# lipku/LiveTalking

Hardware: NVIDIA H100
Metric: lip-sync frames/sec (wav2lip256, 256x256, batch 16, mel + U-Net fwd + paste-back) (higher is better)
Workload: dtype f16 (fp32 accumulate); mel f64; paste u8

## Files before the change

### livetalking_b200/csrc/conv_halo.cu

```cuda
#include <cuda.h>

#include <atomic>
#include <mutex>
#include <utility>

#include "conv_halo.h"
#include "ltb_internal.h"
#include "ptx_sm90.cuh"

#ifdef LTB_HALO_DIAG
#include <cstdlib>
#define LTB_DIAG(bit) (p.dbg & (bit))
#else
#define LTB_DIAG(bit) 0
#endif

namespace ltb {

constexpr int kHaloP = 10;
constexpr int kHaloThreads = 384;
constexpr int kProducerRegs = 40, kConsumerRegs = 232;
constexpr int kSms = 132;

template <int BN, int NSUB, int NACC, int TAPS, int RC = 0>
// ... 477 lines not shown
          bool row_ok = false;
          const size_t opix = halo_pix(img, ty, tx, q >> 1, 0, wq * 16 + (lane >> 2) + 8 * (q & 1), row_ok);
          if (q < 2 * NSUB && row_ok) {
            float ha0 = head_sw[96], ha1 = head_sw[97], ha2 = head_sw[98];
#pragma unroll
            for (int i = 0; i < 4; ++i)
#pragma unroll
              for (int src = 0; src < 4; ++src) {
                const float2 f = __half22float2(*reinterpret_cast<__half2*>(&hv[src][i]));
                const int cc = 8 * i + 2 * src;
                ha0 = fmaf(f.x, head_sw[cc], ha0);
                ha0 = fmaf(f.y, head_sw[cc + 1], ha0);
                ha1 = fmaf(f.x, head_sw[32 + cc], ha1);
                ha1 = fmaf(f.y, head_sw[32 + cc + 1], ha1);
                ha2 = fmaf(f.x, head_sw[64 + cc], ha2);
                ha2 = fmaf(f.y, head_sw[64 + cc + 1], ha2);
              }
            float* o = p.head_out + opix * 3;
            o[0] = (1.f / (1.f + expf(-ha0))) * 255.f;
            o[1] = (1.f / (1.f + expf(-ha1))) * 255.f;
            o[2] = (1.f / (1.f + expf(-ha2))) * 255.f;
          }
        }
      }
    }
  }

  __syncthreads();
  if (gn_smem) {
    for (int i = tid; i < p.gn_images * p.gn_groups * 2; i += kHaloThreads) {
      const float v = gn_acc[i];
      if (v != 0.f) atomicAdd(p.gn_stats + i, v);
    }
  }
}

typedef CUresult (*EncodeTiledFn)(CUtensorMap*, CUtensorMapDataType, cuuint32_t, void*, const cuuint64_t*, const cuuint64_t*,
                                  const cuuint32_t*, const cuuint32_t*, CUtensorMapInterleave, CUtensorMapSwizzle,
                                  CUtensorMapL2promotion, CUtensorMapFloatOOBfill);

static EncodeTiledFn get_encode() {
  static EncodeTiledFn fn = nullptr;
  static std::once_flag once;
  std::call_once(once, []() {
    void* p = nullptr;
    cudaDriverEntryPointQueryResult q;
    if (cudaGetDriverEntryPoint("cuTensorMapEncodeTiled", &p, cudaEnableDefault, &q) == cudaSuccess &&
        q == cudaDriverEntryPointSuccess)
      fn = reinterpret_cast<EncodeTiledFn>(p);
  });
  return fn;
}

static bool encode(CUtensorMap* tm, int rank, const void* base, const cuuint64_t* dims, const cuuint64_t* strides_bytes,
                   const cuuint32_t* box, int spatial_stride = 1) {
  EncodeTiledFn fn = get_encode();
  if (!fn) return false;
  cuuint32_t es[5] = {1, (cuuint32_t)spatial_stride, (cuuint32_t)spatial_stride, 1, 1};
  return fn(tm, CU_TENSOR_MAP_DATA_TYPE_FLOAT16, (cuuint32_t)rank, const_cast<void*>(base), dims, strides_bytes, box, es,
            CU_TENSOR_MAP_INTERLEAVE_NONE, CU_TENSOR_MAP_SWIZZLE_128B, CU_TENSOR_MAP_L2_PROMOTION_L2_256B,
            CU_TENSOR_MAP_FLOAT_OOB_FILL_NONE) == CUDA_SUCCESS;
}

static bool is_conv3x3(const ConvParams& p) {
  if (p.nphases != 1 || p.ph[0].ntaps != 9 || p.sy != 1 || p.sx != 1 || p.osy != 1 || p.osx != 1) return false;
  for (int t = 0; t < 9; ++t)
    if (p.ph[0].dy[t] != t / 3 - 1 || p.ph[0].dx[t] != t % 3 - 1) return false;
  return p.IH == p.GH && p.IW == p.GW && p.OH == p.GH && p.OW == p.GW;
}
static bool is_convT(const ConvParams& p) {
  if (p.nphases != 4 || p.osy != 2 || p.osx != 2 || p.sy != 1 || p.sx != 1) return false;
  const int nt[4] = {1, 2, 2, 4};
  for (int i = 0; i < 4; ++i)
    if (p.ph[i].ntaps != nt[i]) return false;
  return p.IH == p.GH && p.IW == p.GW && p.OH == 2 * p.GH && p.OW == 2 * p.GW;
}

static bool is_conv3x3_s2(const ConvParams& p) {
  if (p.nphases != 1 || p.ph[0].ntaps != 9 || p.sy != 2 || p.sx != 2 || p.osy != 1 || p.osx != 1) return false;
  for (int t = 0; t < 9; ++t)
    if (p.ph[0].dy[t] != t / 3 - 1 || p.ph[0].dx[t] != t % 3 - 1) return false;
  return p.IH == 2 * p.GH && p.IW == 2 * p.GW && p.OH == p.GH && p.OW == p.GW;
}

static bool is_upconv(const ConvParams& p) {
  return p.upconv == 1 && p.nphases == 4 && p.osy == 2 && p.osx == 2 && p.sy == 1 && p.sx == 1 && p.IH == p.GH && p.IW == p.GW &&
         p.OH == 2 * p.GH && p.OW == 2 * p.GW;
}

static bool is_gemm(const ConvParams& p) {
  return p.nphases == 1 && p.ph[0].ntaps == 1 && p.ph[0].dy[0] == 0 && p.ph[0].dx[0] == 0 && p.sy == 1 && p.sx == 1 && p.osy == 1 &&
         p.osx == 1 && p.IH == p.GH && p.IW == p.GW && p.OH == p.GH && p.OW == p.GW;
}

static bool pick_cfg(const ConvParams& p, int* BN, int* NSUB, int* NACC);

bool conv_halo_supported(const ConvParams& p) {
  if (p.zbatch > 1) return false;
  if ((p.OCtot % 8) || (p.oc_off % 8) || (reinterpret_cast<uintptr_t>(p.out) % 16)) return false;
  if (p.res && ((p.RCtot % 8) || (p.rc_off % 8) || (reinterpret_cast<uintptr_t>(p.res) % 16))) return false;
  if (p.group_slot && (!is_gemm(p) || (p.w_slot_stride * 2) % 16 != 0)) return false;
  if (is_gemm(p)) {
    return p.Cout % 32 == 0 && p.Cin % 8 == 0 && p.Cin >= 32 && (p.ICtot % 8) == 0 && (p.ic_off % 8) == 0 && (p.Ktot % 8) == 0 &&
           (p.ph[0].koff % 8) == 0 && p.M >= 512 && get_encode() != nullptr;
  }
  if (is_conv3x3_s2(p)) {
    return p.Cout % 32 == 0 && p.Cin >= 64 && (p.ICtot % 8) == 0 && (p.ic_off % 8) == 0 && p.Ktot == 9 * p.Cin && p.GH >= 16 &&
           p.GW >= 8 && get_encode() != nullptr;
// ... 32 lines not shown
  if (is_conv3x3_s2(p)) {
    *NACC = 1;
    *NSUB = 1;
    *BN = (p.Cout % 64 == 0) ? 64 : 32;
    return true;
  }
  const bool tr = is_convT(p);
  *NACC = tr ? 4 : 1;
  if (tr) {
    *NSUB = 1;
    *BN = (p.Cout % 64 == 0) ? 64 : 32;
    return true;
  }
  const long ksteps = (p.Cin + 15) / 16;
  double best = 1e30;
  for (int bn : {128, 64, 32}) {
    if (p.Cout % bn) continue;
    for (int nsub : {2, 1}) {
      if (nsub == 2 && (p.GH % 32) != 0) continue;
      const long tiles = (long)p.N * ((p.GH + 16 * nsub - 1) / (16 * nsub)) * ((p.GW + 7) / 8) * (p.Cout / bn);
      const long waves = (tiles + kSms - 1) / kSms;
      const double tile = (double)ksteps * 9 * nsub * (55.0 + 0.2 * bn) + 800.0;
      const double epi = (waves == 1) ? 40.0 * nsub * bn : 0.0;
      const double cost = waves * tile + epi;
      if (cost < best * 0.9) {
        best = cost;
        *BN = bn;
        *NSUB = nsub;
      }
    }
  }
  return best < 1e30;
}

int conv_halo_make_plan(const ConvParams& p, const __half* w_tap_major, HaloPlan* out) {
  if (!conv_halo_supported(p)) return 1;
  HaloParams& h = out->hp;
  std::memset(&h, 0, sizeof(h));
  out->grouped = false;
  int BN, NSUB, NACC;
  if (!pick_cfg(p, &BN, &NSUB, &NACC)) return 1;
  out->BN = BN;
  out->NSUB = NSUB;
  out->NACC = NACC;
  const bool up = is_upconv(p);
  const bool s2 = is_conv3x3_s2(p);
  const bool tr = NACC == 4 && !up;
  const bool gemm = is_gemm(p);
  out->TAPS = gemm ? 1 : (up ? 16 : (s2 ? 10 : 9));
  if (gemm) {
    cuuint64_t dims[2] = {(cuuint64_t)p.Cin, (cuuint64_t)p.M};
    cuuint64_t strides[1] = {(cuuint64_t)p.ICtot * 2};
    cuuint32_t box[2] = {64, (cuuint32_t)(128 * NSUB)};
    if (!encode(&h.tm_in, 2, p.in + p.ic_off, dims, strides, box)) return 2;
    cuuint64_t wdims[3] = {(cuuint64_t)p.Cin, (cuuint64_t)p.Cout, (cuuint64_t)p.slots};
    cuuint64_t wstrides[2] = {(cuuint64_t)p.Ktot * 2, (cuuint64_t)p.w_slot_stride * 2};
    cuuint32_t wbox[3] = {64, (cuuint32_t)BN, 1};
    if (!encode(&h.tm_w, p.group_slot ? 3 : 2, p.w + p.ph[0].koff, wdims, wstrides, wbox)) return 2;
  } else
  {
    cuuint64_t dims[4] = {(cuuint64_t)p.Cin, (cuuint64_t)p.IW, (cuuint64_t)p.IH, (cuuint64_t)p.N};
    cuuint64_t strides[3] = {(cuuint64_t)p.ICtot * 2, (cuuint64_t)p.IW * p.ICtot * 2, (cuuint64_t)p.IH * p.IW * p.ICtot * 2};
    cuuint32_t box[4] = {64, (cuuint32_t)kHaloP, (cuuint32_t)(16 * NSUB + 2), 1};
    if (s2) {
      box[1] = 2 * 9 - 1;
      box[2] = 2 * (16 * NSUB + 1) - 1;
    }
    if (!encode(&h.tm_in, 4, p.in + p.ic_off, dims, strides, box, s2 ? 2 : 1)) return 2;
  }
  if (up) {
    cuuint64_t dims[3] = {(cuuint64_t)p.Cin, (cuuint64_t)p.Cout, 16};
    cuuint64_t strides[2] = {(cuuint64_t)p.Cin * 2, (cuuint64_t)p.Cout * p.Cin * 2};
    cuuint32_t box[3] = {64, (cuuint32_t)BN, 4};
    if (!encode(&h.tm_w, 3, w_tap_major, dims, strides, box)) return 2;
  } else if (!gemm) {
    cuuint64_t dims[3] = {(cuuint64_t)p.Cin, (cuuint64_t)p.Cout, 9};
    cuuint64_t strides[2] = {(cuuint64_t)p.Cin * 2, (cuuint64_t)p.Cout * p.Cin * 2};
    cuuint32_t box[3] = {64, (cuuint32_t)BN, 3};
    if (!encode(&h.tm_w, 3, w_tap_major, dims, strides, box)) return 2;
  }
  h.out = p.out;
  h.res = p.res;
  h.bias = p.bias;
  h.N = p.N;
  h.M = p.M;
  h.Cin = p.Cin;
  h.gn_stats = nullptr;
#ifdef LTB_HALO_DIAG
  if (const char* e = std::getenv("LTB_HALO_DIAG")) h.dbg = std::atoi(e);
#endif
  h.OCtot = p.OCtot;
  h.oc_off = p.oc_off;
  h.RCtot = p.RCtot;
  h.rc_off = p.rc_off;
  h.OH = p.OH;
  h.OW = p.OW;
  h.GH = p.GH;
  h.GW = p.GW;
  h.osy = p.osy;
  h.osx = p.osx;
  h.relu = p.relu;
  h.res_halo = halo_res_smem_ok(BN, NSUB, NACC, out->TAPS) && p.res != nullptr && p.res == p.in && p.Cin == p.Cout &&
               p.rc_off == p.ic_off && p.RCtot == p.ICtot;
  h.halo_y0 = tr ? 0 : -1;
  h.halo_x0 = tr ? 0 : -1;
  if (up || tr) {
    const int slot_phase[4] = {0, 1, 3, 2};
    for (int sl = 0; sl < 4; ++sl) {
      h.acc_oy[sl] = p.ph[slot_phase[sl]].ooy;
      h.acc_ox[sl] = p.ph[slot_phase[sl]].oox;
    }
  } else {
    h.acc_oy[0] = p.ph[0].ooy;
    h.acc_ox[0] = p.ph[0].oox;
  }
  h.tiles_n = p.Cout / BN;
  if (gemm) {
    h.halo_y0 = h.halo_x0 = 0;
    h.tiles_x = (p.M + 128 * NSUB - 1) / (128 * NSUB);
    if (p.group_slot) {
      out->grouped = true;
      h.group_slot = p.group_slot;
      h.group_rows = p.group_images * p.GH * p.GW;
      h.group_tiles = (h.group_rows + 128 * NSUB - 1) / (128 * NSUB);
      h.bias_slot_stride = p.bias_slot_stride;
      h.tiles_x = (p.N / p.group_images) * h.group_tiles;
    }
    h.tiles_y = 1;
    h.total_tiles = h.tiles_x * h.tiles_n;
    return 0;
  }
  h.tiles_x = (p.GW + 7) / 8;
// ... 129 lines not shown
```

### livetalking_b200/csrc/conv_halo.h

```cpp
#pragma once
#include <cuda.h>
#include <cuda_runtime.h>

#include <cstring>

#include "conv_params.h"

namespace ltb {

struct alignas(64) HaloParams {
  CUtensorMap tm_in;
  CUtensorMap tm_w;
  __half* out;
  const __half* res;
  const float* bias;
  int N, M, Cin;
  int OCtot, oc_off, RCtot, rc_off;
  int OH, OW, osy, osx;
  int GH, GW;
  int relu;
  int res_halo;
  int halo_y0, halo_x0;
  int acc_oy[4], acc_ox[4];
  int tiles_x, tiles_y, tiles_n, total_tiles;
  float* gn_stats;
  int gn_groups, gn_cpg, gn_hw, gn_images;
  const float* head_w;
  const float* head_b;
  float* head_out;
  const int* group_slot;
  int group_rows, group_tiles;
  long long bias_slot_stride;
#ifdef LTB_HALO_DIAG
  int dbg;
#endif
};

struct HaloPlan {
  HaloParams hp;
  int BN, NSUB, NACC, TAPS;
  bool grouped;
};

bool conv_halo_supported(const ConvParams& p);
int conv_halo_make_plan(const ConvParams& p, const __half* w_tap_major, HaloPlan* out);
cudaError_t launch_conv_halo(const HaloPlan& pl, cudaStream_t st);
int conv_halo_sms();
int conv_halo_resident_chunks(const HaloPlan& pl, int sms);
bool conv_halo_gn_fusable(const HaloPlan& pl, int cout_total, int groups, int hw);
cudaError_t launch_w_tap_major(const __half* w, __half* wt, int cout, int cin, cudaStream_t st, int ntaps = 9);
cudaError_t launch_w_tap_major_convT(const __half* w, __half* wt, int cout, int cin, cudaStream_t st);

}
```

### livetalking_b200/csrc/conv_plan.cu

```cuda
#include <cstring>
#include <string>
#include <vector>

#include "../../include/ltb200.h"
#include "conv_plan.h"
#include "ltb_internal.h"

namespace ltb {

static const int kTd[2][2] = {{0, 0}, {0, 1}};
static const int kTk[2][2] = {{1, 0}, {2, 0}};
static const int kTn[2] = {1, 2};
static const int kUd[2][2] = {{-1, 0}, {0, 1}};

ConvParams conv_params(ConvMode mode, int N, ConvSlice in, int IH, int IW, int Cin, ConvSlice out, int OH, int OW, int Cout,
                       ConvSlice res, const __half* w, int Ktot, int w_koff, const float* bias, bool relu, ConvTaps taps) {
  ConvParams p;
  std::memset(&p, 0, sizeof(p));
  p.in = in.p;
  p.N = N;
  p.IH = IH;
  p.IW = IW;
  p.ICtot = in.Ctot;
  p.ic_off = in.off;
// ... 8 lines not shown
  p.Cout = Cout;
  p.res = res.p;
  p.RCtot = res.Ctot;
  p.rc_off = res.off;
  p.w = w;
  p.Ktot = Ktot;
  p.bias = bias;
  p.relu = relu ? 1 : 0;
  if (mode == ConvMode::Dense) {
    p.sy = taps.sy;
    p.sx = taps.sx;
    p.GH = OH;
    p.GW = OW;
    p.nphases = 1;
    ConvPhase& ph = p.ph[0];
    ph.ntaps = taps.KH * taps.KW;
    ph.koff = w_koff;
    for (int kh = 0; kh < taps.KH; ++kh)
      for (int kw = 0; kw < taps.KW; ++kw) {
        ph.dy[kh * taps.KW + kw] = (signed char)(kh - taps.pad_t);
        ph.dx[kh * taps.KW + kw] = (signed char)(kw - taps.pad_l);
      }
  } else {
    const bool up = mode == ConvMode::Upsample2x;
    p.GH = IH;
    p.GW = IW;
    p.osy = p.osx = 2;
    p.nphases = 4;
    p.upconv = up ? 1 : 0;
    int koff = w_koff;
    for (int a = 0; a < 2; ++a)
      for (int b = 0; b < 2; ++b) {
        ConvPhase& ph = p.ph[a * 2 + b];
        const int na = up ? 2 : kTn[a], nb = up ? 2 : kTn[b];
        ph.ntaps = na * nb;
        ph.koff = koff;
        ph.ooy = a;
        ph.oox = b;
        for (int i = 0; i < na; ++i)
          for (int j = 0; j < nb; ++j) {
            ph.dy[i * nb + j] = (signed char)(up ? kUd[a][i] : kTd[a][i]);
            ph.dx[i * nb + j] = (signed char)(up ? kUd[b][j] : kTd[b][j]);
          }
        koff += ph.ntaps * Cin;
      }
  }
  p.M = N * p.GH * p.GW;
  return p;
}

int conv_plan(const ConvParams& p, const __half* w_tap, ConvPath path, ConvPlan* out) {
  out->p = p;
  out->halo = false;
  if (p.group_slot) {
    if (p.group_images < 1 || p.N % p.group_images || p.slots < 1 || p.w_slot_stride < 0 || p.bias_slot_stride < 0)
      return LTB_FAIL("conv: grouped weights need N divisible by group_images >= 1, slots >= 1 and non-negative slot strides");
    if (p.zbatch > 1 || p.upconv) return LTB_FAIL("conv: grouped weights cannot be combined with zbatch or the fused upsample");
  }
  if (path == ConvPath::Gather) return 0;
  const bool gemm = p.nphases == 1 && p.ph[0].ntaps == 1;
  if (!((w_tap || gemm) && conv_halo_supported(p))) {
    if (path == ConvPath::Auto) return 0;
    return LTB_FAIL("conv: the halo kernel cannot run " + std::to_string(p.N) + "x" + std::to_string(p.IH) + "x" + std::to_string(p.IW) +
                    "x" + std::to_string(p.Cin) + " -> " + std::to_string(p.OH) + "x" + std::to_string(p.OW) + "x" + std::to_string(p.Cout) +
                    (w_tap || gemm ? "" : " without tap-major weights"));
  }
  if (conv_halo_make_plan(p, w_tap, &out->hp) != 0) return LTB_FAIL("conv: halo plan / tensor map creation failed");
  out->halo = true;
  return 0;
}

cudaError_t conv_launch(const ConvPlan& pl, cudaStream_t st, float* splitk_ws, size_t ws_floats) {
  return pl.halo ? launch_conv_halo(pl.hp, st) : launch_conv_gather(pl.p, st, splitk_ws, ws_floats);
}

bool conv_plan_variant(const ConvPlan& pl, bool have_ws, size_t ws_floats, ltb_conv_variant* out) {
  std::memset(out, 0, sizeof(*out));
  out->grouped = pl.p.group_slot != nullptr;
  if (pl.halo) {
    out->kernel = 1;
    out->taps = pl.hp.TAPS;
    out->bn = pl.hp.BN;
    out->nsub = pl.hp.NSUB;
    out->nacc = pl.hp.NACC;
    out->resident_chunks = conv_halo_resident_chunks(pl.hp, conv_halo_sms());
    out->res_halo = pl.hp.hp.res_halo;
    return true;
  }
  int ksplit = 0;
  if (!conv_gather_pick(pl.p, have_ws, ws_floats, &out->bn, &out->kb, &ksplit)) return false;
  out->ksplit = ksplit > 1 ? ksplit : 1;
  return true;
}

bool conv_plan_fuse_gn_stats(ConvPlan* pl, float* stats, int groups, int hw) {
  const ConvParams& p = pl->p;
  if (!pl->halo || pl->hp.grouped || p.oc_off != 0 || p.OCtot != p.Cout || !conv_halo_gn_fusable(pl->hp, p.Cout, groups, hw)) return false;
  HaloParams& h = pl->hp.hp;
  h.gn_stats = stats;
  h.gn_groups = groups;
  h.gn_cpg = p.Cout / groups;
  h.gn_hw = hw;
  h.gn_images = p.M / hw;
  return true;
}

bool conv_plan_fuse_head(ConvPlan* pl, const float* w, const float* b, float* out) {
  if (!pl->halo || pl->hp.grouped || pl->hp.BN != 32 || pl->p.Cout != 32) return false;
  pl->hp.hp.head_w = w;
  pl->hp.hp.head_b = b;
  pl->hp.hp.head_out = out;
  return true;
}

static void pack_conv_w(const float* w, int cout, int cin, int KH, int KW, std::vector<__half>& out) {
  out.resize((size_t)cout * KH * KW * cin);
  for (int co = 0; co < cout; ++co)
    for (int kh = 0; kh < KH; ++kh)
      for (int kw = 0; kw < KW; ++kw)
        for (int ci = 0; ci < cin; ++ci)
          out[((size_t)co * KH * KW + kh * KW + kw) * cin + ci] = __float2half(w[(((size_t)co * cin + ci) * KH + kh) * KW + kw]);
}
static void pack_convT_w(const float* w, int cin, int cout, std::vector<__half>& out) {
  out.resize((size_t)cout * 9 * cin);
  for (int co = 0; co < cout; ++co) {
    size_t k = 0;
    for (int a = 0; a < 2; ++a)
      for (int b = 0; b < 2; ++b)
        for (int i = 0; i < kTn[a]; ++i)
          for (int j = 0; j < kTn[b]; ++j) {
            const int kh = kTk[a][i], kw = kTk[b][j];
// ... 28 lines not shown
  }
  if (OH <= 0 || OW <= 0) return LTB_FAIL("empty output");
  const size_t in_b = (size_t)d->N * d->IH * d->IW * d->Cin * 2, out_b = (size_t)d->N * OH * OW * d->Cout * 2;
  __half *din = nullptr, *dout = nullptr, *dw = nullptr, *dres = nullptr, *dwt = nullptr;
  float* dbias = nullptr;
  float* dws = nullptr;
  cudaEvent_t e0 = nullptr, e1 = nullptr;
  int rc = 0;
  auto cleanup = [&]() {
    cudaFree(din);
    cudaFree(dout);
    cudaFree(dw);
    cudaFree(dres);
    cudaFree(dwt);
    cudaFree(dws);
    cudaFree(dbias);
    if (e0) cudaEventDestroy(e0);
    if (e1) cudaEventDestroy(e1);
  };
#define CK(x)                                                             \
  do {                                                                    \
    cudaError_t _e = (x);                                                 \
    if (_e != cudaSuccess) {                                              \
      rc = LTB_FAIL(std::string(#x) + ": " + cudaGetErrorString(_e));     \
      cleanup();                                                          \
      return rc;                                                          \
    }                                                                     \
  } while (0)
  CK(cudaMalloc(&din, in_b));
  CK(cudaMalloc(&dout, out_b));
  CK(cudaMalloc(&dw, wp.size() * 2));
  CK(cudaMalloc(&dbias, (size_t)d->Cout * 4));
  CK(cudaMemcpy(din, in_f16, in_b, cudaMemcpyHostToDevice));
  CK(cudaMemcpy(dw, wp.data(), wp.size() * 2, cudaMemcpyHostToDevice));
  CK(cudaMemcpy(dbias, bias_f32, (size_t)d->Cout * 4, cudaMemcpyHostToDevice));
  CK(cudaMemset(dout, 0xFF, out_b));
  if (d->has_res) {
    CK(cudaMalloc(&dres, out_b));
    CK(cudaMemcpy(dres, res_f16, out_b, cudaMemcpyHostToDevice));
  }
  if (d->KH == 3 && d->KW == 3) {
    CK(cudaMalloc(&dwt, wp.size() * 2));
    CK(d->transposed ? launch_w_tap_major_convT(dw, dwt, d->Cout, d->Cin, nullptr) : launch_w_tap_major(dw, dwt, d->Cout, d->Cin, nullptr));
  }
  const ConvParams p = conv_params(d->transposed ? ConvMode::Transposed : ConvMode::Dense, d->N, {din, d->Cin, 0}, d->IH, d->IW, d->Cin,
                                   {dout, d->Cout, 0}, OH, OW, d->Cout, d->has_res ? ConvSlice{dres, d->Cout, 0} : ConvSlice{}, dw, Ktot, 0,
                                   dbias, d->relu != 0, {d->KH, d->KW, d->sy, d->sx, d->pad, d->pad});
  const ConvPath path = d->force_path == 1 ? ConvPath::Gather : d->force_path == 2 ? ConvPath::Halo : ConvPath::Auto;
  ConvPlan pl;
  if (conv_plan(p, dwt, path, &pl)) {
    cleanup();
    return 1;
  }
  const size_t ws_floats = pl.halo ? 0 : (size_t)1 << 22;
  if (ws_floats) {
    CK(cudaMalloc(&dws, ws_floats * sizeof(float)));
    CK(cudaMemset(dws, 0, ws_floats * sizeof(float)));
  }
  CK(conv_launch(pl, nullptr, dws, ws_floats));
  if (reps > 0) {
    CK(cudaEventCreate(&e0));
    CK(cudaEventCreate(&e1));
    for (int i = 0; i < 3; ++i) CK(conv_launch(pl, nullptr, dws, ws_floats));
    CK(cudaEventRecord(e0, nullptr));
    for (int i = 0; i < reps; ++i) CK(conv_launch(pl, nullptr, dws, ws_floats));
    CK(cudaEventRecord(e1, nullptr));
    CK(cudaEventSynchronize(e1));
    CK(cudaEventElapsedTime(ms_out, e0, e1));
    *ms_out /= reps;
  }
  CK(cudaDeviceSynchronize());
  CK(cudaMemcpy(out_f16, dout, out_b, cudaMemcpyDeviceToHost));
#undef CK
  cleanup();
  return 0;
}

extern "C" {

int ltb_conv2d_f16(const ltb_conv_desc* d, const void* in_f16, const float* w_f32, const float* bias_f32,
                   const void* res_f16, void* out_f16) {
  return conv2d_f16_impl(d, in_f16, w_f32, bias_f32, res_f16, out_f16, 0, nullptr);
}

int ltb_conv2d_f16_timed(const ltb_conv_desc* d, const void* in_f16, const float* w_f32, const float* bias_f32,
                         const void* res_f16, void* out_f16, int reps, float* ms_per_launch) {
  if (reps < 1 || !ms_per_launch) return LTB_FAIL("conv2d_f16_timed: reps >= 1 and a result pointer are required");
  return conv2d_f16_impl(d, in_f16, w_f32, bias_f32, res_f16, out_f16, reps, ms_per_launch);
}

}
```

### livetalking_b200/csrc/conv_plan.h

```cpp
#pragma once
#include <cuda_runtime.h>

#include "conv_halo.h"

struct ltb_conv_variant;

namespace ltb {

struct ConvSlice {
  const __half* p;
  int Ctot, off;
};

enum class ConvMode {
  Dense,
  Transposed,
  Upsample2x,
};
struct ConvTaps {
  int KH, KW, sy, sx, pad_t, pad_l;
};

inline int conv_out_dim(int in, int k, int s, int pad) { return (in + 2 * pad - k) / s + 1; }

ConvParams conv_params(ConvMode mode, int N, ConvSlice in, int IH, int IW, int Cin, ConvSlice out, int OH, int OW, int Cout,
                       ConvSlice res, const __half* w, int Ktot, int w_koff, const float* bias, bool relu, ConvTaps taps = {});

enum class ConvPath {
  Auto,
  Gather,
  Halo,
};
struct ConvPlan {
  ConvParams p{};
  bool halo = false;
  HaloPlan hp{};
};

int conv_plan(const ConvParams& p, const __half* w_tap, ConvPath path, ConvPlan* out);
cudaError_t conv_launch(const ConvPlan& pl, cudaStream_t st, float* splitk_ws, size_t ws_floats);
bool conv_plan_variant(const ConvPlan& pl, bool have_ws, size_t ws_floats, ltb_conv_variant* out);

bool conv_plan_fuse_gn_stats(ConvPlan* pl, float* stats, int groups, int hw);
bool conv_plan_fuse_head(ConvPlan* pl, const float* w, const float* b, float* out);

}
```

### livetalking_b200/csrc/ptx_sm90.cuh

```cuda
#pragma once
#include <cuda_fp16.h>
#include <cstdint>
#include <cstdio>

namespace ltb {

__device__ __forceinline__ uint32_t smem_u32(const void* p) {
  return static_cast<uint32_t>(__cvta_generic_to_shared(p));
}

__device__ __forceinline__ void mbar_init(uint32_t bar, uint32_t count) {
  asm volatile("mbarrier.init.shared::cta.b64 [%0], %1;" ::"r"(bar), "r"(count) : "memory");
}
__device__ __forceinline__ void mbar_fence_init() {
  asm volatile("fence.mbarrier_init.release.cluster;" ::: "memory");
}
__device__ __forceinline__ void mbar_arrive(uint32_t bar) {
  asm volatile("mbarrier.arrive.shared::cta.b64 _, [%0];" ::"r"(bar) : "memory");
}
__device__ __forceinline__ void mbar_arrive_expect_tx(uint32_t bar, uint32_t bytes) {
  asm volatile("mbarrier.arrive.expect_tx.shared::cta.b64 _, [%0], %1;" ::"r"(bar), "r"(bytes) : "memory");
}
__device__ __forceinline__ bool mbar_try_wait(uint32_t bar, uint32_t parity) {
  uint32_t ok;
// ... 18 lines not shown
  asm volatile("fence.proxy.async.shared::cta;" ::: "memory");
}

__device__ __forceinline__ void cp_async16(uint32_t dst, const void* src, uint32_t src_bytes) {
  asm volatile("cp.async.cg.shared.global [%0], [%1], 16, %2;" ::"r"(dst), "l"(src), "r"(src_bytes) : "memory");
}
__device__ __forceinline__ void cp_async_commit() { asm volatile("cp.async.commit_group;" ::: "memory"); }
template <int N>
__device__ __forceinline__ void cp_async_wait() {
  asm volatile("cp.async.wait_group %0;" ::"n"(N) : "memory");
}
__device__ __forceinline__ uint4 lds128(uint32_t addr) {
  uint4 v;
  asm volatile("ld.shared.v4.u32 {%0, %1, %2, %3}, [%4];" : "=r"(v.x), "=r"(v.y), "=r"(v.z), "=r"(v.w) : "r"(addr) : "memory");
  return v;
}

__device__ __forceinline__ void tma_prefetch_desc(const void* tmap) {
  asm volatile("prefetch.tensormap [%0];" ::"l"(tmap) : "memory");
}
__device__ __forceinline__ void tma_load_2d(uint32_t dst, const void* tmap, uint32_t bar, int c0, int c1) {
  asm volatile(
      "cp.async.bulk.tensor.2d.shared::cluster.global.mbarrier::complete_tx::bytes [%0], [%1, {%3, %4}], [%2];" ::"r"(dst),
      "l"(tmap), "r"(bar), "r"(c0), "r"(c1)
      : "memory");
}
__device__ __forceinline__ void tma_load_3d(uint32_t dst, const void* tmap, uint32_t bar, int c0, int c1, int c2) {
  asm volatile(
      "cp.async.bulk.tensor.3d.shared::cluster.global.mbarrier::complete_tx::bytes [%0], [%1, {%3, %4, %5}], [%2];" ::"r"(dst),
      "l"(tmap), "r"(bar), "r"(c0), "r"(c1), "r"(c2)
      : "memory");
}
__device__ __forceinline__ void tma_load_4d(uint32_t dst, const void* tmap, uint32_t bar, int c0, int c1, int c2, int c3) {
  asm volatile(
      "cp.async.bulk.tensor.4d.shared::cluster.global.mbarrier::complete_tx::bytes [%0], [%1, {%3, %4, %5, %6}], [%2];" ::"r"(
          dst),
      "l"(tmap), "r"(bar), "r"(c0), "r"(c1), "r"(c2), "r"(c3)
      : "memory");
}
__device__ __forceinline__ void tma_load_5d(uint32_t dst, const void* tmap, uint32_t bar, int c0, int c1, int c2, int c3,
                                            int c4) {
  asm volatile(
      "cp.async.bulk.tensor.5d.shared::cluster.global.mbarrier::complete_tx::bytes [%0], [%1, {%3, %4, %5, %6, %7}], [%2];" ::
          "r"(dst),
      "l"(tmap), "r"(bar), "r"(c0), "r"(c1), "r"(c2), "r"(c3), "r"(c4)
      : "memory");
}

__device__ __forceinline__ void ldmatrix_x4(uint32_t& r0, uint32_t& r1, uint32_t& r2, uint32_t& r3, uint32_t saddr) {
  asm volatile("ldmatrix.sync.aligned.m8n8.x4.shared.b16 {%0, %1, %2, %3}, [%4];"
               : "=r"(r0), "=r"(r1), "=r"(r2), "=r"(r3)
               : "r"(saddr)
               : "memory");
}

__device__ __forceinline__ uint64_t wgmma_desc(uint32_t saddr, uint32_t lbo_bytes, uint32_t sbo_bytes, uint32_t layout) {
  uint64_t d = 0;
  d |= (uint64_t)((saddr & 0x3FFFF) >> 4);
  d |= (uint64_t)((lbo_bytes >> 4) & 0x3FFF) << 16;
  d |= (uint64_t)((sbo_bytes >> 4) & 0x3FFF) << 32;
  d |= (uint64_t)(layout & 3) << 62;
  return d;
}
__host__ __device__ constexpr uint32_t wgmma_hi_128b(uint32_t sbo_bytes) { return (sbo_bytes >> 4) | (1u << 30); }
__device__ __forceinline__ uint32_t wgmma_lo(uint32_t saddr) { return ((saddr & 0x3FFFFu) >> 4) | (1u << 16); }
__device__ __forceinline__ uint64_t wgmma_lohi(uint32_t lo, uint32_t hi) { return ((uint64_t)hi << 32) | lo; }

__device__ __forceinline__ void wgmma_fence() { asm volatile("wgmma.fence.sync.aligned;" ::: "memory"); }
__device__ __forceinline__ void wgmma_commit() { asm volatile("wgmma.commit_group.sync.aligned;" ::: "memory"); }
template <int N>
__device__ __forceinline__ void wgmma_wait() {
  asm volatile("wgmma.wait_group.sync.aligned %0;" ::"n"(N) : "memory");
}
template <int R>
__device__ __forceinline__ void wgmma_fence_regs(float (&d)[R]) {
#pragma unroll
  for (int i = 0; i < R; ++i) asm volatile("" : "+f"(d[i])::"memory");
}

template <int N>
struct Wgmma;
#define LTB_D1(i) "+f"(d[i])
#define LTB_D2(i) LTB_D1(i), LTB_D1(i + 1)
#define LTB_D4(i) LTB_D2(i), LTB_D2(i + 2)
#define LTB_D8(i) LTB_D4(i), LTB_D4(i + 4)
#define LTB_D16(i) LTB_D8(i), LTB_D8(i + 8)
#define LTB_D32(i) LTB_D16(i), LTB_D16(i + 16)
#define LTB_D64(i) LTB_D32(i), LTB_D32(i + 32)
#define LTB_D128(i) LTB_D64(i), LTB_D64(i + 64)
#define LTB_WG_HEAD(P) "{\n.reg .pred p;\nsetp.ne.b32 p, %" P ", 0;\nwgmma.mma_async.sync.aligned.m64n"
#define LTB_WG_SS(N, REGS, A, B, P) LTB_WG_HEAD(P) N "k16.f32.f16.f16 " REGS ", %" A ", %" B ", p, 1, 1, 0, 0;\n}\n"
#define LTB_WG_RS(N, REGS, A, B, P) \
  LTB_WG_HEAD(P) N "k16.f32.f16.f16 " REGS ", {%" A "}, %" B ", p, 1, 1, 0;\n}\n"

template <>
struct Wgmma<16> {
#define LTB_R "{%0,%1,%2,%3,%4,%5,%6,%7}"
  __device__ __forceinline__ static void ss(float (&d)[8], uint64_t a, uint64_t b, uint32_t acc) {
    asm volatile(LTB_WG_SS("16", LTB_R, "8", "9", "10") : LTB_D8(0) : "l"(a), "l"(b), "r"(acc));
  }
  __device__ __forceinline__ static void rs(float (&d)[8], const uint32_t (&a)[4], uint64_t b, uint32_t acc) {
    asm volatile(LTB_WG_RS("16", LTB_R, "8,%9,%10,%11", "12", "13") : LTB_D8(0)
                 : "r"(a[0]), "r"(a[1]), "r"(a[2]), "r"(a[3]), "l"(b), "r"(acc));
  }
#undef LTB_R
};
// ... 162 lines not shown
```

### livetalking_b200/csrc/w2l_engine.cu

```cuda
#include <cstring>
#include <memory>
#include <mutex>
#include <string>
#include <vector>

#include "../../include/ltb200.h"
#include "conv_plan.h"
#include "ltb_internal.h"
#include "stem_umma.h"

namespace ltb {

static thread_local std::string g_last_error;
void set_error(const std::string& msg) { g_last_error = msg; }

bool pdl_default() {
  static const bool on = [] {
    const char* e = std::getenv("LTB_NO_PDL");
    return !(e && e[0] && e[0] != '0');
  }();
  return on;
}
static thread_local int g_pdl = -1;
bool pdl_enabled() { return g_pdl < 0 ? pdl_default() : g_pdl == 1; }
// ... 240 lines not shown
  const int catS[8] = {512, 512, 512, 256, 128, 64, 32, 16};
  __half* cat[8];
  for (int i = 0; i < 8; ++i) {
    void* p;
    if (dev_alloc(s, (size_t)B * catH[i] * catH[i] * (catD[i] + catS[i]) * 2, &p, true)) return 1;
    cat[i] = static_cast<__half*>(p);
  }
  const size_t tmp_bytes = (size_t)B * 256 * 256 * 64 * 2;
  __half* ring[2] = {nullptr, nullptr};
  int ring_next = 0;
  auto new_tmp = [&](int H, int W, int C, View* v) -> int {
    void* p = nullptr;
    if (keep) {
      if (dev_alloc(s, (size_t)B * H * W * C * 2, &p, true)) return 1;
    } else {
      if (!ring[ring_next]) {
        if (dev_alloc(s, tmp_bytes, &p, true)) return 1;
        ring[ring_next] = static_cast<__half*>(p);
      }
      p = ring[ring_next];
      ring_next ^= 1;
    }
    *v = View{static_cast<__half*>(p), H, W, C, 0, C};
    return 0;
  };
  __half* aring[2] = {nullptr, nullptr};
  int aring_next = 0;
  auto new_atmp = [&](int H, int W, int C, View* v) -> int {
    void* p = nullptr;
    if (keep) {
      if (dev_alloc(s, (size_t)B * H * W * C * 2, &p, true)) return 1;
    } else {
      if (!aring[aring_next]) {
        if (dev_alloc(s, (size_t)B * 80 * 16 * 32 * 2, &p, true)) return 1;
        aring[aring_next] = static_cast<__half*>(p);
      }
      p = aring[aring_next];
      aring_next ^= 1;
    }
    *v = View{static_cast<__half*>(p), H, W, C, 0, C};
    return 0;
  };
  auto cat_dec = [&](int i) { return View{cat[i], catH[i], catH[i], catD[i] + catS[i], 0, catD[i]}; };
  auto cat_skip = [&](int i) { return View{cat[i], catH[i], catH[i], catD[i] + catS[i], catD[i], catS[i]}; };
  auto cat_all = [&](int i) { return View{cat[i], catH[i], catH[i], catD[i] + catS[i], 0, catD[i] + catS[i]}; };

  auto record = [&](int li, const View& v) {
    s->louts[li] = LayerOut{v.p, v.H, v.W, v.C, v.Ctot, v.c_off};
  };
  const ConvPath path = (s->flags & LTB_SESSION_NO_HALO) ? ConvPath::Gather : ConvPath::Auto;
  auto push_conv = [&](int li, const ConvParams& p) -> int {
    Op o;
    if (conv_plan(p, m->wt[li], path, &o.conv)) return LTB_FAIL("plan: layer " + std::to_string(li) + ": " + g_last_error);
    o.type = o.conv.halo ? 4 : 0;
    s->ops.push_back(o);
    return 0;
  };
  auto add_conv = [&](int li, const View& in, const View& out, const View* res) -> int {
    const LDef& L = kLayers[li];
    if (in.C != L.cin || out.C != L.cout) return LTB_FAIL("plan: channel mismatch at layer " + std::to_string(li));
    const int OH = conv_out_dim(in.H, L.k, L.sy, L.pad), OW = conv_out_dim(in.W, L.k, L.sx, L.pad);
    if (OH != out.H || OW != out.W) return LTB_FAIL("plan: spatial mismatch at layer " + std::to_string(li));
    const ConvParams p = conv_params(ConvMode::Dense, B, in.slice(), in.H, in.W, L.cin, out.slice(), OH, OW, L.cout,
                                     res ? res->slice() : ConvSlice{}, m->w[li], L.k * L.k * L.cin, 0, m->bias[li], true,
                                     {L.k, L.k, L.sy, L.sx, L.pad, L.pad});
    if (push_conv(li, p)) return 1;
    record(li, out);
    return 0;
  };
  auto add_convT = [&](int li, const View& in, const View& out) -> int {
    const LDef& L = kLayers[li];
    if (in.C != L.cin || out.C != L.cout || out.H != 2 * in.H) return LTB_FAIL("plan: convT mismatch at layer " + std::to_string(li));
    const ConvParams p = conv_params(ConvMode::Transposed, B, in.slice(), in.H, in.W, L.cin, out.slice(), out.H, out.W, L.cout,
                                     ConvSlice{}, m->w[li], 9 * L.cin, 0, m->bias[li], true);
    if (push_conv(li, p)) return 1;
    record(li, out);
    return 0;
  };

  {
    Op o;
    o.type = 6;
    o.branch = 1;
    s->ops.push_back(o);
  }
  View a_prev;
  if (new_atmp(80, 16, 32, &a_prev)) return 1;
  {
    Op o;
    o.type = 2;
    o.audio_out = a_prev.p;
    o.branch = 1;
    s->ops.push_back(o);
    record(0, a_prev);
  }
  {
    int H = 80, W = 16;
    for (int li = 1; li <= 12; ++li) {
      const LDef& L = kLayers[li];
      const int OH = conv_out_dim(H, L.k, L.sy, L.pad), OW = conv_out_dim(W, L.k, L.sx, L.pad);
      View o;
      if (new_atmp(OH, OW, L.cout, &o)) return 1;
      if (add_conv(li, a_prev, o, L.res ? &a_prev : nullptr)) return 1;
      s->ops.back().branch = 1;
      a_prev = o;
      H = OH;
      W = OW;
// ... 750 lines not shown
```

Before: 6880.

## Add ping-pong warpgroup kernel for 64-channel residual 3x3 convs

Adds a specialized persistent kernel for stride-1 3x3 convolutions with 64 input and output channels and an in-place residual. Two consumer warpgroups alternate tiles, ordered by named barriers, so one warpgroup's epilogue overlaps the other's WGMMA. The weights stay resident in shared memory, inputs come through a 4-stage TMA ring, and outputs are written back with TMA stores after stmatrix. The residual is read from the halo tile already in shared memory rather than from global memory. It is on by default for eligible layers and adds a new code path with tight shape constraints and custom synchronisation that must be correct.

```diff
diff --git a/livetalking_b200/csrc/conv_halo.cu b/livetalking_b200/csrc/conv_halo.cu
--- a/livetalking_b200/csrc/conv_halo.cu
+++ b/livetalking_b200/csrc/conv_halo.cu
@@ -553,8 +553,8 @@
   return fn;
 }
 
-static bool encode(CUtensorMap* tm, int rank, const void* base, const cuuint64_t* dims, const cuuint64_t* strides_bytes,
-                   const cuuint32_t* box, int spatial_stride = 1) {
+bool encode_tmap_f16(CUtensorMap* tm, int rank, const void* base, const cuuint64_t* dims, const cuuint64_t* strides_bytes,
+                     const cuuint32_t* box, int spatial_stride) {
   EncodeTiledFn fn = get_encode();
   if (!fn) return false;
   cuuint32_t es[5] = {1, (cuuint32_t)spatial_stride, (cuuint32_t)spatial_stride, 1, 1};
@@ -693,11 +693,11 @@
     cuuint64_t dims[2] = {(cuuint64_t)p.Cin, (cuuint64_t)p.M};
     cuuint64_t strides[1] = {(cuuint64_t)p.ICtot * 2};
     cuuint32_t box[2] = {64, (cuuint32_t)(128 * NSUB)};
-    if (!encode(&h.tm_in, 2, p.in + p.ic_off, dims, strides, box)) return 2;
+    if (!encode_tmap_f16(&h.tm_in, 2, p.in + p.ic_off, dims, strides, box)) return 2;
     cuuint64_t wdims[3] = {(cuuint64_t)p.Cin, (cuuint64_t)p.Cout, (cuuint64_t)p.slots};
     cuuint64_t wstrides[2] = {(cuuint64_t)p.Ktot * 2, (cuuint64_t)p.w_slot_stride * 2};
     cuuint32_t wbox[3] = {64, (cuuint32_t)BN, 1};
-    if (!encode(&h.tm_w, p.group_slot ? 3 : 2, p.w + p.ph[0].koff, wdims, wstrides, wbox)) return 2;
+    if (!encode_tmap_f16(&h.tm_w, p.group_slot ? 3 : 2, p.w + p.ph[0].koff, wdims, wstrides, wbox)) return 2;
   } else
   {
     cuuint64_t dims[4] = {(cuuint64_t)p.Cin, (cuuint64_t)p.IW, (cuuint64_t)p.IH, (cuuint64_t)p.N};
@@ -707,18 +707,18 @@
       box[1] = 2 * 9 - 1;
       box[2] = 2 * (16 * NSUB + 1) - 1;
     }
-    if (!encode(&h.tm_in, 4, p.in + p.ic_off, dims, strides, box, s2 ? 2 : 1)) return 2;
+    if (!encode_tmap_f16(&h.tm_in, 4, p.in + p.ic_off, dims, strides, box, s2 ? 2 : 1)) return 2;
   }
   if (up) {
     cuuint64_t dims[3] = {(cuuint64_t)p.Cin, (cuuint64_t)p.Cout, 16};
     cuuint64_t strides[2] = {(cuuint64_t)p.Cin * 2, (cuuint64_t)p.Cout * p.Cin * 2};
     cuuint32_t box[3] = {64, (cuuint32_t)BN, 4};
-    if (!encode(&h.tm_w, 3, w_tap_major, dims, strides, box)) return 2;
+    if (!encode_tmap_f16(&h.tm_w, 3, w_tap_major, dims, strides, box)) return 2;
   } else if (!gemm) {
     cuuint64_t dims[3] = {(cuuint64_t)p.Cin, (cuuint64_t)p.Cout, 9};
     cuuint64_t strides[2] = {(cuuint64_t)p.Cin * 2, (cuuint64_t)p.Cout * p.Cin * 2};
     cuuint32_t box[3] = {64, (cuuint32_t)BN, 3};
-    if (!encode(&h.tm_w, 3, w_tap_major, dims, strides, box)) return 2;
+    if (!encode_tmap_f16(&h.tm_w, 3, w_tap_major, dims, strides, box)) return 2;
   }
   h.out = p.out;
   h.res = p.res;
diff --git a/livetalking_b200/csrc/conv_halo.h b/livetalking_b200/csrc/conv_halo.h
--- a/livetalking_b200/csrc/conv_halo.h
+++ b/livetalking_b200/csrc/conv_halo.h
@@ -45,6 +45,8 @@
 bool conv_halo_supported(const ConvParams& p);
 int conv_halo_make_plan(const ConvParams& p, const __half* w_tap_major, HaloPlan* out);
 cudaError_t launch_conv_halo(const HaloPlan& pl, cudaStream_t st);
+bool encode_tmap_f16(CUtensorMap* tm, int rank, const void* base, const cuuint64_t* dims, const cuuint64_t* strides_bytes,
+                     const cuuint32_t* box, int spatial_stride = 1);
 int conv_halo_sms();
 int conv_halo_resident_chunks(const HaloPlan& pl, int sms);
 bool conv_halo_gn_fusable(const HaloPlan& pl, int cout_total, int groups, int hw);
diff --git a/livetalking_b200/csrc/conv_pingpong.cu b/livetalking_b200/csrc/conv_pingpong.cu
--- /dev/null
+++ b/livetalking_b200/csrc/conv_pingpong.cu
@@ -0,0 +1,210 @@
+#include <cuda.h>
+
+#include <cstdlib>
+#include <cstring>
+
+#include "conv_halo.h"
+#include "conv_pingpong.h"
+#include "ltb_internal.h"
+#include "ptx_sm90.cuh"
+
+namespace ltb {
+
+namespace {
+
+constexpr int kThreads = 384;
+constexpr int kProducerRegs = 40, kConsumerRegs = 232;
+constexpr int kP = 10, kHR = 18;
+constexpr int kStages = 4;
+constexpr int kABytesRaw = kHR * kP * 128;
+constexpr int kABytes = (kABytesRaw + 1023) & ~1023;
+constexpr int kTapBytes = 64 * 128;
+constexpr int kWBytes = 9 * kTapBytes;
+constexpr int kOutBytes = 128 * 128;
+constexpr int kSmemBytes = kWBytes + kStages * kABytes + 2 * kOutBytes + 1024;
+static_assert(kSmemBytes + 1024 <= 227 * 1024, "shared memory overflow");
+constexpr uint32_t kBarOrder = 1, kBarStage = 3;
+
+}
+
+__global__ void __launch_bounds__(kThreads, 1) conv_pingpong_kernel(const __grid_constant__ PingpongParams p) {
+  extern __shared__ uint8_t smem_raw[];
+  __shared__ __align__(8) uint64_t a_full[kStages], a_empty[kStages], w_full;
+  const int tid = threadIdx.x, warp = tid >> 5, lane = tid & 31;
+  const uint32_t smem0 = (smem_u32(smem_raw) + 1023u) & ~1023u;
+  const uint32_t w_smem = smem0;
+  const uint32_t a_smem = w_smem + kWBytes;
+  const uint32_t o_smem = a_smem + kStages * kABytes;
+  const int tiles_img = p.tiles_x * p.tiles_y;
+
+  if (tid == 0) {
+    for (int s = 0; s < kStages; ++s) {
+      mbar_init(smem_u32(&a_full[s]), 1);
+      mbar_init(smem_u32(&a_empty[s]), 4);
+    }
+    mbar_init(smem_u32(&w_full), 1);
+    mbar_fence_init();
+    tma_prefetch_desc(&p.tm_in);
+    tma_prefetch_desc(&p.tm_w);
+    tma_prefetch_desc(&p.tm_out);
+  }
+  __syncthreads();
+
+  pdl_launch_dependents();
+  if (warp == 8 && lane == 0) {
+    mbar_arrive_expect_tx(smem_u32(&w_full), kWBytes);
+    for (int j = 0; j < 3; ++j) tma_load_3d(w_smem + 3 * j * kTapBytes, &p.tm_w, smem_u32(&w_full), 0, 0, 3 * j);
+  }
+  pdl_wait();
+
+  if (warp >= 8) {
+    setmaxnreg_dec<kProducerRegs>();
+    if (warp == 8 && lane == 0) {
+      uint32_t s = 0;
+      for (int t = blockIdx.x; t < p.total_tiles; t += gridDim.x, ++s) {
+        const int img = t / tiles_img, r = t - img * tiles_img;
+        const int ty = r / p.tiles_x, tx = r - ty * p.tiles_x;
+        const uint32_t st = s % kStages;
+        mbar_wait(smem_u32(&a_empty[st]), ((s / kStages) & 1u) ^ 1u);
+        mbar_arrive_expect_tx(smem_u32(&a_full[st]), kABytesRaw);
+        tma_load_4d(a_smem + st * kABytes, &p.tm_in, smem_u32(&a_full[st]), 0, tx * 8 - 1, ty * 16 - 1, img);
+      }
+    }
+    return;
+  }
+
+  setmaxnreg_inc<kConsumerRegs>();
+  const int wg = warp >> 2, wq = warp & 3;
+  const bool leader = (tid & 127) == 0;
+  const uint32_t obuf = o_smem + wg * kOutBytes;
+  constexpr uint32_t kWHi = wgmma_hi_128b(1024);
+  constexpr uint32_t kXHi = wgmma_hi_128b(kP * 128);
+  const uint32_t w_lo0 = wgmma_lo(w_smem);
+  const int c0 = 16 * wq + (lane >> 2);
+  const float bias0 = __ldg(p.bias + c0), bias1 = __ldg(p.bias + c0 + 8);
+  const __half2 hmax = __floats2half2_rn(65504.f, 65504.f);
+  const __half2 hlo = p.relu ? __floats2half2_rn(0.f, 0.f) : __floats2half2_rn(-65504.f, -65504.f);
+  const int lm_row = lane >> 4, lm_cb = 2 * wq + ((lane >> 3) & 1), lm_x = lane & 7;
+  mbar_wait(smem_u32(&w_full), 0);
+
+  uint32_t s = wg;
+  for (int t = blockIdx.x + wg * gridDim.x; t < p.total_tiles; t += 2 * gridDim.x, s += 2) {
+    const int img = t / tiles_img, r = t - img * tiles_img;
+    const int ty = r / p.tiles_x, tx = r - ty * p.tiles_x;
+    const uint32_t st = s % kStages;
+    const uint32_t abase = a_smem + st * kABytes;
+    if (s > 0) named_sync(kBarOrder + wg, 256);
+    mbar_wait(smem_u32(&a_full[st]), (s / kStages) & 1u);
+
+    uint32_t rh[16][2];
+#pragma unroll
+    for (int i = 0; i < 16; i += 2) {
+      const int hr = (i + lm_row + 1) * kP + lm_x + 1;
+      ldmatrix_x4_trans(rh[i][0], rh[i][1], rh[i + 1][0], rh[i + 1][1], abase + hr * 128 + ((lm_cb ^ (hr & 7)) << 4));
+    }
+
+    float acc[64];
+#pragma unroll
+    for (int i = 0; i < 64; ++i) acc[i] = 0.f;
+    const uint32_t x_lo0 = wgmma_lo(abase);
+    wgmma_fence();
+#pragma unroll
+    for (int j = 0; j < 3; ++j)
+#pragma unroll
+      for (int k = 0; k < 4; ++k)
+#pragma unroll
+        for (int tt = 0; tt < 3; ++tt)
+          Wgmma<128>::ss(acc, wgmma_lohi(w_lo0 + (3 * j + tt) * (kTapBytes / 16) + k * 2, kWHi),
+                         wgmma_lohi(x_lo0 + (j * kP + tt) * 8 + k * 2, kXHi), 1u);
+    wgmma_commit();
+    if (t + gridDim.x < p.total_tiles) named_arrive(kBarOrder + (wg ^ 1), 256);
+    wgmma_wait<0>();
+    wgmma_fence_regs(acc);
+    __syncwarp();
+    if (lane == 0) mbar_arrive(smem_u32(&a_empty[st]));
+
+    if (leader) bulk_wait_read<0>();
+    named_sync(kBarStage + wg, 128);
+    auto out2 = [&](float f0, float f1, float b, uint32_t res) {
+      const uint32_t v = f32x2_to_f16x2_sat(f0 + b, f1 + b);
+      const __half2 o = __hmin2(__hmax2(__hadd2(*reinterpret_cast<const __half2*>(&v), *reinterpret_cast<const __half2*>(&res)), hlo), hmax);
+      return *reinterpret_cast<const uint32_t*>(&o);
+    };
+#pragma unroll
+    for (int i = 0; i < 16; i += 2) {
+      const uint32_t o0 = out2(acc[4 * i], acc[4 * i + 1], bias0, rh[i][0]);
+      const uint32_t o1 = out2(acc[4 * i + 2], acc[4 * i + 3], bias1, rh[i][1]);
+      const uint32_t o2 = out2(acc[4 * i + 4], acc[4 * i + 5], bias0, rh[i + 1][0]);
+      const uint32_t o3 = out2(acc[4 * i + 6], acc[4 * i + 7], bias1, rh[i + 1][1]);
+      stmatrix_x4_trans(obuf + ((i + lm_row) * 8 + lm_x) * 128 + ((lm_cb ^ lm_x) << 4), o0, o1, o2, o3);
+    }
+    fence_proxy_async_smem();
+    named_sync(kBarStage + wg, 128);
+    if (leader) {
+      tma_store_4d(&p.tm_out, obuf, 0, tx * 8, ty * 16, img);
+      bulk_commit();
+    }
+  }
+  if (leader) bulk_wait<0>();
+}
+
+static bool pingpong_enabled() {
+  const char* e = std::getenv("LTB_CONV_PINGPONG");
+  return !(e && std::strcmp(e, "0") == 0);
+}
+
+bool conv_pingpong_supported(const ConvParams& p) {
+  if (p.zbatch > 1 || p.group_slot || p.upconv || p.nphases != 1 || p.ph[0].ntaps != 9) return false;
+  if (p.sy != 1 || p.sx != 1 || p.osy != 1 || p.osx != 1) return false;
+  for (int t = 0; t < 9; ++t)
+    if (p.ph[0].dy[t] != t / 3 - 1 || p.ph[0].dx[t] != t % 3 - 1) return false;
+  if (p.IH != p.GH || p.IW != p.GW || p.OH != p.GH || p.OW != p.GW) return false;
+  if (p.Cin != 64 || p.Cout != 64 || p.Ktot != 9 * 64) return false;
+  if (p.res != p.in || p.rc_off != p.ic_off || p.RCtot != p.ICtot) return false;
+  if ((p.ICtot % 8) || (p.ic_off % 8) || (p.OCtot % 8) || (p.oc_off % 8) || (reinterpret_cast<uintptr_t>(p.out) % 16) ||
+      (reinterpret_cast<uintptr_t>(p.in) % 16))
+    return false;
+  if (p.GW % 8) return false;
+  const long tiles = (long)p.N * ((p.GH + 15) / 16) * ((p.GW + 7) / 8);
+  if (tiles < 3L * conv_halo_sms()) return false;
+  return pingpong_enabled();
+}
+
+int conv_pingpong_make_plan(const ConvParams& p, const __half* w_tap_major, PingpongParams* out) {
+  if (!conv_pingpong_supported(p) || !w_tap_major) return 1;
+  std::memset(out, 0, sizeof(*out));
+  {
+    const cuuint64_t dims[4] = {64, (cuuint64_t)p.IW, (cuuint64_t)p.IH, (cuuint64_t)p.N};
+    const cuuint64_t strides[3] = {(cuuint64_t)p.ICtot * 2, (cuuint64_t)p.IW * p.ICtot * 2, (cuuint64_t)p.IH * p.IW * p.ICtot * 2};
+    const cuuint32_t box[4] = {64, kP, kHR, 1};
+    if (!encode_tmap_f16(&out->tm_in, 4, p.in + p.ic_off, dims, strides, box)) return 2;
+  }
+  {
+    const cuuint64_t dims[3] = {64, 64, 9};
+    const cuuint64_t strides[2] = {64 * 2, 64 * 64 * 2};
+    const cuuint32_t box[3] = {64, 64, 3};
+    if (!encode_tmap_f16(&out->tm_w, 3, w_tap_major, dims, strides, box)) return 2;
+  }
+  {
+    const cuuint64_t dims[4] = {64, (cuuint64_t)p.OW, (cuuint64_t)p.OH, (cuuint64_t)p.N};
+    const cuuint64_t strides[3] = {(cuuint64_t)p.OCtot * 2, (cuuint64_t)p.OW * p.OCtot * 2, (cuuint64_t)p.OH * p.OW * p.OCtot * 2};
+    const cuuint32_t box[4] = {64, 8, 16, 1};
+    if (!encode_tmap_f16(&out->tm_out, 4, p.out + p.oc_off, dims, strides, box)) return 2;
+  }
+  out->bias = p.bias;
+  out->relu = p.relu;
+  out->tiles_x = (p.GW + 7) / 8;
+  out->tiles_y = (p.GH + 15) / 16;
+  out->total_tiles = out->tiles_x * out->tiles_y * p.N;
+  return 0;
+}
+
+cudaError_t launch_conv_pingpong(const PingpongParams& pp, cudaStream_t st) {
+  static SmemConfigOnce once;
+  if (cudaError_t e = once.ensure(conv_pingpong_kernel, kSmemBytes); e != cudaSuccess) return e;
+  const int sms = conv_halo_sms();
+  const int grid = pp.total_tiles < sms ? pp.total_tiles : sms;
+  return launch_kernel_pdl(conv_pingpong_kernel, dim3(grid), dim3(kThreads), kSmemBytes, st, pp);
+}
+
+}
diff --git a/livetalking_b200/csrc/conv_pingpong.h b/livetalking_b200/csrc/conv_pingpong.h
--- /dev/null
+++ b/livetalking_b200/csrc/conv_pingpong.h
@@ -0,0 +1,22 @@
+#pragma once
+#include <cuda.h>
+#include <cuda_runtime.h>
+
+#include "conv_params.h"
+
+namespace ltb {
+
+struct alignas(64) PingpongParams {
+  CUtensorMap tm_in;
+  CUtensorMap tm_w;
+  CUtensorMap tm_out;
+  const float* bias;
+  int relu;
+  int tiles_x, tiles_y, total_tiles;
+};
+
+bool conv_pingpong_supported(const ConvParams& p);
+int conv_pingpong_make_plan(const ConvParams& p, const __half* w_tap_major, PingpongParams* out);
+cudaError_t launch_conv_pingpong(const PingpongParams& pp, cudaStream_t st);
+
+}
diff --git a/livetalking_b200/csrc/conv_plan.cu b/livetalking_b200/csrc/conv_plan.cu
--- a/livetalking_b200/csrc/conv_plan.cu
+++ b/livetalking_b200/csrc/conv_plan.cu
@@ -84,12 +84,18 @@
 int conv_plan(const ConvParams& p, const __half* w_tap, ConvPath path, ConvPlan* out) {
   out->p = p;
   out->halo = false;
+  out->pingpong = false;
   if (p.group_slot) {
     if (p.group_images < 1 || p.N % p.group_images || p.slots < 1 || p.w_slot_stride < 0 || p.bias_slot_stride < 0)
       return LTB_FAIL("conv: grouped weights need N divisible by group_images >= 1, slots >= 1 and non-negative slot strides");
     if (p.zbatch > 1 || p.upconv) return LTB_FAIL("conv: grouped weights cannot be combined with zbatch or the fused upsample");
   }
   if (path == ConvPath::Gather) return 0;
+  if (w_tap && conv_pingpong_supported(p)) {
+    if (conv_pingpong_make_plan(p, w_tap, &out->pp) != 0) return LTB_FAIL("conv: ping-pong plan / tensor map creation failed");
+    out->pingpong = true;
+    return 0;
+  }
   const bool gemm = p.nphases == 1 && p.ph[0].ntaps == 1;
   if (!((w_tap || gemm) && conv_halo_supported(p))) {
     if (path == ConvPath::Auto) return 0;
@@ -103,12 +109,23 @@
 }
 
 cudaError_t conv_launch(const ConvPlan& pl, cudaStream_t st, float* splitk_ws, size_t ws_floats) {
+  if (pl.pingpong) return launch_conv_pingpong(pl.pp, st);
   return pl.halo ? launch_conv_halo(pl.hp, st) : launch_conv_gather(pl.p, st, splitk_ws, ws_floats);
 }
 
 bool conv_plan_variant(const ConvPlan& pl, bool have_ws, size_t ws_floats, ltb_conv_variant* out) {
   std::memset(out, 0, sizeof(*out));
   out->grouped = pl.p.group_slot != nullptr;
+  if (pl.pingpong) {
+    out->kernel = 2;
+    out->taps = 9;
+    out->bn = 64;
+    out->nsub = 1;
+    out->nacc = 1;
+    out->resident_chunks = 1;
+    out->res_halo = 1;
+    return true;
+  }
   if (pl.halo) {
     out->kernel = 1;
     out->taps = pl.hp.TAPS;
@@ -243,7 +260,7 @@
     cleanup();
     return 1;
   }
-  const size_t ws_floats = pl.halo ? 0 : (size_t)1 << 22;
+  const size_t ws_floats = (pl.halo || pl.pingpong) ? 0 : (size_t)1 << 22;
   if (ws_floats) {
     CK(cudaMalloc(&dws, ws_floats * sizeof(float)));
     CK(cudaMemset(dws, 0, ws_floats * sizeof(float)));
diff --git a/livetalking_b200/csrc/conv_plan.h b/livetalking_b200/csrc/conv_plan.h
--- a/livetalking_b200/csrc/conv_plan.h
+++ b/livetalking_b200/csrc/conv_plan.h
@@ -2,6 +2,7 @@
 #include <cuda_runtime.h>
 
 #include "conv_halo.h"
+#include "conv_pingpong.h"
 
 struct ltb_conv_variant;
 
@@ -35,6 +36,8 @@
   ConvParams p{};
   bool halo = false;
   HaloPlan hp{};
+  bool pingpong = false;
+  PingpongParams pp{};
 };
 
 int conv_plan(const ConvParams& p, const __half* w_tap, ConvPath path, ConvPlan* out);
diff --git a/livetalking_b200/csrc/ptx_sm90.cuh b/livetalking_b200/csrc/ptx_sm90.cuh
--- a/livetalking_b200/csrc/ptx_sm90.cuh
+++ b/livetalking_b200/csrc/ptx_sm90.cuh
@@ -94,6 +94,39 @@
                : "=r"(r0), "=r"(r1), "=r"(r2), "=r"(r3)
                : "r"(saddr)
                : "memory");
+}
+
+__device__ __forceinline__ void ldmatrix_x4_trans(uint32_t& r0, uint32_t& r1, uint32_t& r2, uint32_t& r3, uint32_t saddr) {
+  asm volatile("ldmatrix.sync.aligned.m8n8.x4.trans.shared.b16 {%0, %1, %2, %3}, [%4];"
+               : "=r"(r0), "=r"(r1), "=r"(r2), "=r"(r3)
+               : "r"(saddr)
+               : "memory");
+}
+__device__ __forceinline__ void stmatrix_x4_trans(uint32_t saddr, uint32_t r0, uint32_t r1, uint32_t r2, uint32_t r3) {
+  asm volatile("stmatrix.sync.aligned.m8n8.x4.trans.shared.b16 [%0], {%1, %2, %3, %4};" ::"r"(saddr), "r"(r0), "r"(r1), "r"(r2), "r"(r3)
+               : "memory");
+}
+
+__device__ __forceinline__ void tma_store_4d(const void* tmap, uint32_t src, int c0, int c1, int c2, int c3) {
+  asm volatile("cp.async.bulk.tensor.4d.global.shared::cta.bulk_group [%0, {%2, %3, %4, %5}], [%1];" ::"l"(tmap), "r"(src), "r"(c0),
+               "r"(c1), "r"(c2), "r"(c3)
+               : "memory");
+}
+__device__ __forceinline__ void bulk_commit() { asm volatile("cp.async.bulk.commit_group;" ::: "memory"); }
+template <int N>
+__device__ __forceinline__ void bulk_wait_read() {
+  asm volatile("cp.async.bulk.wait_group.read %0;" ::"n"(N) : "memory");
+}
+template <int N>
+__device__ __forceinline__ void bulk_wait() {
+  asm volatile("cp.async.bulk.wait_group %0;" ::"n"(N) : "memory");
+}
+
+__device__ __forceinline__ void named_sync(uint32_t id, uint32_t threads) {
+  asm volatile("bar.sync %0, %1;" ::"r"(id), "r"(threads) : "memory");
+}
+__device__ __forceinline__ void named_arrive(uint32_t id, uint32_t threads) {
+  asm volatile("bar.arrive %0, %1;" ::"r"(id), "r"(threads) : "memory");
 }
 
 __device__ __forceinline__ uint64_t wgmma_desc(uint32_t saddr, uint32_t lbo_bytes, uint32_t sbo_bytes, uint32_t layout) {
diff --git a/livetalking_b200/csrc/w2l_engine.cu b/livetalking_b200/csrc/w2l_engine.cu
--- a/livetalking_b200/csrc/w2l_engine.cu
+++ b/livetalking_b200/csrc/w2l_engine.cu
@@ -316,7 +316,7 @@
   auto push_conv = [&](int li, const ConvParams& p) -> int {
     Op o;
     if (conv_plan(p, m->wt[li], path, &o.conv)) return LTB_FAIL("plan: layer " + std::to_string(li) + ": " + g_last_error);
-    o.type = o.conv.halo ? 4 : 0;
+    o.type = (o.conv.halo || o.conv.pingpong) ? 4 : 0;
     s->ops.push_back(o);
     return 0;
   };
```

After: 7272 (median of 6 runs). 5.7% higher.
